# wizyoung/YOLOv3_TensorFlow

Hardware: NVIDIA H100
Metric: images/sec (higher is better)
Workload: dtype f16

## Files before the change

### include/yolob200.h

```cpp
#ifndef YOLOB200_H_
#define YOLOB200_H_

#include <stddef.h>
#include <stdint.h>

#ifdef __cplusplus
extern "C" {
#endif

typedef enum yb_status {
  YB_OK = 0,
  YB_ERR_INVALID_ARGUMENT = -1,
  YB_ERR_CUDA = -2,
  YB_ERR_UNSUPPORTED = -3,
  YB_ERR_WORKSPACE = -4
} yb_status;

typedef enum yb_dtype { YB_F16 = 0, YB_BF16 = 1, YB_F32 = 2, YB_E4M3 = 3 } yb_dtype;

typedef enum yb_wlayout {
  YB_W_HWIO = 0,
  YB_W_OIHW = 1,
  YB_W_OHWI = 2
} yb_wlayout;

int yb_version(void);
const char* yb_last_error_string(void);
int yb_set_option(const char* key, const char* value);
const char* yb_get_option(const char* key);
int yb_device_info(int* sm_count, int* cc_major, int* cc_minor);

typedef struct yb_conv_desc {
  int n, h, w;
  int cin, cout;
  int ksize;
  int stride;
  int in_ld;
  int out_ld;
  int res_ld;
  int dtype;
  int out_fp32;
  int leaky;
  int upsample2x;
} yb_conv_desc;

int yb_conv2d_fwd(const yb_conv_desc* d, const void* x, const void* w_packed, const float* scale,
                  const float* shift, const void* res, void* out, float* stat_sum, float* stat_sqsum,
                  void* stream);
int yb_conv_cout_pad(int cout);
int yb_conv2d_fwd_e4m3(const yb_conv_desc* d, const void* x, const void* w_packed, const float* scale,
                       const float* shift, const void* res, float res_scale, void* out, float out_scale, void* stream);
typedef struct yb_conv_schedule_info {
  int pingpong;
  int consumers;
  int cluster;
  int block_m, block_n, block_k;
  int stages;
  int num_kb;
  int num_m_tiles, num_n_tiles;
  int grid;
  int res_smem;
  int res_stages;
  int cluster_m;
  int cluster_n;
  int units;
  int epi_tma;
} yb_conv_schedule_info;
int yb_conv_schedule(const yb_conv_desc* d, int kh, int kw, int with_stats, int sm_count, yb_conv_schedule_info* info);

int yb_stem_conv_fwd(const float* x, const float* w_ohwi, const float* scale, const float* shift, int n, int h,
                     int w, int cout, int dtype, int leaky, void* out, void* stream);

int yb_conv3x3_thin_fwd(const yb_conv_desc* d, const void* x, const void* w_packed, const float* scale,
                        const float* shift, const void* res, void* out, void* stream);
int yb_stem_conv_fwd_tc(const float* x, const float* w_ohwi, const float* scale, const float* shift, int n, int h,
                        int w, int dtype, int leaky, void* out, void* stream);
int yb_stem_conv_fwd_tc_stats(const float* x, const float* w_ohwi, const float* scale, const float* shift, int n, int h,
                              int w, int dtype, int leaky, void* out, float* stat_sum, float* stat_sqsum, void* stream);

int yb_conv3x3_halo_supported(const yb_conv_desc* d);
int yb_conv3x3_halo_fwd(const yb_conv_desc* d, const void* x, const void* w_packed, const float* scale,
                        const float* shift, const void* res, void* out, void* stream);
int yb_stem_conv1_fused_fwd(const yb_conv_desc* d, const float* image, const float* stem_w_ohwi, const float* stem_scale,
                            const float* stem_shift, const void* w_packed, const float* scale, const float* shift, void* out,
                            void* stream);

int yb_process_box(const float* boxes, const int32_t* labels, const int32_t* counts, int n, int vmax, int img_w,
                   int img_h, int class_num, const float* anchors9x2, float* y_true_1, float* y_true_2,
                   float* y_true_3, void* stream);
int yb_letterbox_params(int src_h, int src_w, int new_h, int new_w, double* resize_ratio, int* resize_h, int* resize_w,
                        int* dh, int* dw);
int yb_letterbox_normalize(const uint8_t* bgr, int src_h, int src_w, long src_pitch_bytes, int new_h, int new_w,
                           float* out_rgb, void* stream);
int yb_resize_batch(const uint8_t* images, long images_bytes, const int64_t* desc_host, const int64_t* desc_dev, int n,
                    int new_h, int new_w, int letterbox, int interp, float* out_rgb, double* params, void* stream);
int yb_resize_boxes(float* boxes, const int32_t* counts, int n, int vmax, int box_ld, const int64_t* desc_dev, int new_h,
                    int new_w, int letterbox, void* stream);
int yb_restore_boxes(float* boxes, const int32_t* counts, int n, int slots, int box_ld, const double* params,
                     void* stream);

int yb_pack_conv_weights(const float* src, int layout, int cout, int cin, int ksize, int cout_pad, int dtype,
                         void* dst, void* stream);
int yb_pack_conv_weights_e4m3(const float* src, int layout, int cout, int cin, int ksize, int cout_pad, void* dst,
                              float* w_scale, void* stream);
int yb_amax(const void* x, long ld, long rows, int cols, int dtype, float* out, void* stream);
int yb_bn_fold(const float* gamma, const float* beta, const float* mean, const float* var, int c, float eps,
               float* scale, float* shift, void* stream);

int yb_conv2d_wgrad(const yb_conv_desc* d, const void* x, const void* dz, int dz_ld, int dz_dilated, float* dw,
                    void* stream);
int yb_stem_conv_wgrad(const float* x, const void* dz, int dtype, int n, int h, int w, float* dw, void* stream);
int yb_stem_conv_wgrad_tc(const float* x, const void* dz, int dtype, int n, int h, int w, float* dw, void* stream);
int yb_pack_dgrad_weights(const float* w_ohwi, int cout, int cin, int ksize, int k_cout, int cin_pad, int dtype,
                          void* dst, void* stream);
int yb_pack_dgrad_weights_s2(const float* w_ohwi, int cout, int cin, int k_cout, int cin_pad, int dtype, void* dst,
                             void* stream);
int yb_conv2d_dgrad_s2(const yb_conv_desc* fwd, const void* dz, int dz_ld, int k_cout, const void* w_dgrad_s2,
                       const void* res, int res_ld, void* dx, int dx_ld, void* stream);
typedef struct yb_wgrad_schedule_info {
  int bnw;
  int tp;
  int stages;
  int num_kb;
  int kb_per_split;
  int splits;
  int tiles;
  int grid_x, grid_y, grid_z;
} yb_wgrad_schedule_info;
int yb_wgrad_schedule(const yb_conv_desc* d, int sm_count, yb_wgrad_schedule_info* info);
int yb_bn_finalize(const float* sum, const float* sqsum, long count, int c, const float* gamma, const float* beta,
                   float eps, float decay, float* moving_mean, float* moving_var, float* scale, float* shift,
                   float* save_mean, float* save_invstd, void* stream);
int yb_bn_act_apply(const void* z, long z_ld, const float* scale, const float* shift, const void* res, long res_ld,
                    void* out, long out_ld, int n, int h, int w, int c, int dtype, int leaky, int upsample2x,
                    void* stream);
int yb_bn_stats_act_apply(const void* z, long z_ld, const float* sum, const float* sqsum, const float* gamma,
                          const float* beta, float eps, float decay, float* moving_mean, float* moving_var,
                          float* scale, float* shift, float* save_mean, float* save_invstd, const void* res,
                          long res_ld, void* out, long out_ld, int n, int h, int w, int c, int dtype, int leaky,
                          int upsample2x, void* stream);
typedef struct yb_bn_schedule_info {
  int cpt;
  int r;
  int blocks_per_sm;
  int cv;
  int lanes;
  long rows_per_block;
  int grid;
} yb_bn_schedule_info;
int yb_bn_schedule(long rows, int c, int sm_count, yb_bn_schedule_info* info);
int yb_bn_bwd_reduce_workspace_bytes(size_t* bytes);
// ... 178 lines not shown
```

### yolov3_tensorflow_b200/_lib.py

```python
from __future__ import annotations

import ctypes as C
import os

_HERE = os.path.dirname(os.path.abspath(__file__))
LIB_PATH = os.path.join(_HERE, "libyolob200.so")

YB_F16, YB_BF16, YB_F32, YB_E4M3 = 0, 1, 2, 3
YB_W_HWIO, YB_W_OIHW, YB_W_OHWI = 0, 1, 2
YB_OPT_SGD, YB_OPT_MOMENTUM, YB_OPT_RMSPROP, YB_OPT_ADAM = 0, 1, 2, 3
YB_TRAIN_FORWARD_ONLY, YB_TRAIN_BN_FROZEN, YB_TRAIN_NO_BACKWARD = 1, 2, 4
YB_PHASE_LOCAL, YB_PHASE_GLOBAL = 0, 1
YB_VOC_MAX_GT = 1024
YB_KMEANS_MAX_K = 32
YB_JPEG_BAD_MARKER, YB_JPEG_BAD_RST, YB_JPEG_BAD_CODE, YB_JPEG_BAD_INDEX, YB_JPEG_TRUNCATED = 1, 2, 4, 8, 16
YB_LAYER_IGEMM, YB_LAYER_HALO, YB_LAYER_FUSED_STEM, YB_LAYER_STEM, YB_LAYER_THIN = 1, 2, 3, 4, 5


class YoloB200Error(RuntimeError):
    pass


if not os.path.exists(LIB_PATH):
    raise ImportError(
        f"{LIB_PATH} not found: build it with ./build.sh (or python -c 'import __graft_entry__ as g; g.build()'). "
        "yolov3_tensorflow_b200 has no CPU/PyTorch fallback.")

lib = C.CDLL(LIB_PATH)

vp, i32, f32, sz = C.c_void_p, C.c_int, C.c_float, C.c_size_t


class ConvDesc(C.Structure):
    _fields_ = [(n, i32) for n in ("n", "h", "w", "cin", "cout", "ksize", "stride", "in_ld", "out_ld", "res_ld",
                                   "dtype", "out_fp32", "leaky", "upsample2x")]


class ConvSchedule(C.Structure):
    _fields_ = [(n, i32) for n in ("pingpong", "consumers", "cluster", "block_m", "block_n", "block_k", "stages", "num_kb",
                                   "num_m_tiles", "num_n_tiles", "grid", "res_smem", "res_stages", "cluster_m",
                                   "cluster_n", "units", "epi_tma")]


class LayerSchedule(C.Structure):
    _fields_ = [(n, i32) for n in ("igemm", "pingpong", "cluster_m", "cluster_n", "block_m", "block_n", "num_m_tiles",
                                   "num_n_tiles", "units", "max_clusters", "grid", "residual", "res_smem", "kernel",
                                   "epi_tma", "det_block_n")]


class WgradSchedule(C.Structure):
    _fields_ = [(n, i32) for n in ("bnw", "tp", "stages", "num_kb", "kb_per_split", "splits", "tiles", "grid_x",
                                   "grid_y", "grid_z")]


class BnSchedule(C.Structure):
    _fields_ = [(n, i32) for n in ("cpt", "r", "blocks_per_sm", "cv", "lanes")] + [("rows_per_block", C.c_long),
                                                                                    ("grid", i32)]


class LayerInfo(C.Structure):
    _fields_ = [(n, i32) for n in ("index", "cin", "cout", "ksize", "stride", "has_bn", "in_h", "in_w", "out_h",
                                   "out_w", "is_head", "scope_index", "upsample2x")]


class JpegInfo(C.Structure):
    _fields_ = [(n, i32) for n in ("height", "width", "src_height", "src_width", "components", "h_samp", "v_samp",
                                   "restart_interval", "orientation", "mode")]


class Optimizer(C.Structure):
    _fields_ = [("kind", i32)] + [(n, f32) for n in ("lr", "grad_scale", "momentum", "decay", "beta1", "beta2", "epsilon",
                                                      "weight_decay", "clip_norm")]


_SIGS = {
    "yb_version": ([], i32),
    "yb_last_error_string": ([], C.c_char_p),
    "yb_set_option": ([C.c_char_p, C.c_char_p], i32),
    "yb_get_option": ([C.c_char_p], C.c_char_p),
    "yb_device_info": ([C.POINTER(i32)] * 3, i32),
    "yb_conv2d_fwd": ([C.POINTER(ConvDesc), vp, vp, vp, vp, vp, vp, vp, vp, vp], i32),
    "yb_conv2d_fwd_e4m3": ([C.POINTER(ConvDesc), vp, vp, vp, vp, vp, f32, vp, f32, vp], i32),
    "yb_conv_cout_pad": ([i32], i32),
    "yb_conv_schedule": ([C.POINTER(ConvDesc), i32, i32, i32, i32, C.POINTER(ConvSchedule)], i32),
    "yb_stem_conv_fwd": ([vp, vp, vp, vp, i32, i32, i32, i32, i32, i32, vp, vp], i32),
    "yb_conv3x3_thin_fwd": ([C.POINTER(ConvDesc), vp, vp, vp, vp, vp, vp, vp], i32),
    "yb_conv3x3_halo_supported": ([C.POINTER(ConvDesc)], i32),
    "yb_conv3x3_halo_fwd": ([C.POINTER(ConvDesc), vp, vp, vp, vp, vp, vp, vp], i32),
    "yb_stem_conv1_fused_fwd": ([C.POINTER(ConvDesc), vp, vp, vp, vp, vp, vp, vp, vp, vp], i32),
    "yb_stem_conv_fwd_tc": ([vp, vp, vp, vp, i32, i32, i32, i32, i32, vp, vp], i32),
    "yb_stem_conv_fwd_tc_stats": ([vp, vp, vp, vp, i32, i32, i32, i32, i32, vp, vp, vp, vp], i32),
    "yb_process_box": ([vp, vp, vp, i32, i32, i32, i32, i32, C.POINTER(f32), vp, vp, vp, vp], i32),
    "yb_letterbox_params": ([i32, i32, i32, i32, C.POINTER(C.c_double), C.POINTER(i32), C.POINTER(i32), C.POINTER(i32), C.POINTER(i32)], i32),
    "yb_letterbox_normalize": ([vp, i32, i32, C.c_long, i32, i32, vp, vp], i32),
    "yb_resize_batch": ([vp, C.c_long, vp, vp, i32, i32, i32, i32, i32, vp, vp, vp], i32),
    "yb_resize_boxes": ([vp, vp, i32, i32, i32, vp, i32, i32, i32, vp], i32),
    "yb_restore_boxes": ([vp, vp, i32, i32, i32, vp, vp], i32),
    "yb_pack_conv_weights": ([vp, i32, i32, i32, i32, i32, i32, vp, vp], i32),
    "yb_pack_conv_weights_e4m3": ([vp, i32, i32, i32, i32, i32, vp, vp, vp], i32),
    "yb_amax": ([vp, C.c_long, C.c_long, i32, i32, vp, vp], i32),
    "yb_bn_fold": ([vp, vp, vp, vp, i32, f32, vp, vp, vp], i32),
    "yb_conv2d_wgrad": ([C.POINTER(ConvDesc), vp, vp, i32, i32, vp, vp], i32),
    "yb_stem_conv_wgrad": ([vp, vp, i32, i32, i32, i32, vp, vp], i32),
    "yb_stem_conv_wgrad_tc": ([vp, vp, i32, i32, i32, i32, vp, vp], i32),
    "yb_pack_dgrad_weights": ([vp, i32, i32, i32, i32, i32, i32, vp, vp], i32),
    "yb_pack_dgrad_weights_s2": ([vp, i32, i32, i32, i32, i32, vp, vp], i32),
    "yb_conv2d_dgrad_s2": ([vp, vp, i32, i32, vp, vp, i32, vp, i32, vp], i32),
    "yb_bn_finalize": ([vp, vp, C.c_long, i32, vp, vp, f32, f32, vp, vp, vp, vp, vp, vp, vp], i32),
    "yb_bn_act_apply": ([vp, C.c_long, vp, vp, vp, C.c_long, vp, C.c_long, i32, i32, i32, i32, i32, i32, i32, vp], i32),
    "yb_wgrad_schedule": ([C.POINTER(ConvDesc), i32, C.POINTER(WgradSchedule)], i32),
    "yb_bn_stats_act_apply": ([vp, C.c_long, vp, vp, vp, vp, f32, f32, vp, vp, vp, vp, vp, vp, vp, C.c_long, vp, C.c_long,
                               i32, i32, i32, i32, i32, i32, i32, vp], i32),
    "yb_bn_schedule": ([C.c_long, i32, i32, C.POINTER(BnSchedule)], i32),
    "yb_bn_bwd_reduce_workspace_bytes": ([C.POINTER(sz)], i32),
    "yb_bn_bwd_reduce": ([vp, C.c_long, vp, C.c_long, vp, vp, vp, vp, i32, i32, i32, i32, i32, i32, i32, vp, vp, vp, vp], i32),
    "yb_bn_bwd_apply": ([vp, C.c_long, vp, C.c_long, vp, vp, vp, vp, vp, vp, vp, i32, i32, i32, i32, i32, i32, i32, i32, vp, C.c_long, vp], i32),
    "yb_col_sum": ([vp, C.c_long, C.c_long, i32, i32, vp, vp], i32),
    "yb_col_stats": ([vp, C.c_long, C.c_long, i32, i32, vp, vp, vp], i32),
    "yb_reorg_layer": ([vp, i32, i32, i32, i32, i32, i32, C.POINTER(f32), vp, vp, vp, vp, vp], i32),
    "yb_predict": ([vp, vp, vp, i32, i32, i32, i32, C.POINTER(f32), vp, vp, vp, vp, vp], i32),
    "yb_nms_workspace_bytes": ([i32, i32, i32, i32, C.POINTER(sz)], i32),
    "yb_nms": ([vp, vp, i32, i32, i32, i32, f32, f32, vp, sz, vp, vp, vp, vp, vp, vp], i32),
    "yb_voc_match": ([vp, vp, vp, vp, i32, i32, vp, vp, vp, i32, i32, C.c_double, vp, C.c_long, C.c_long, vp, vp], i32),
    "yb_voc_ap_workspace_bytes": ([C.c_long, i32, C.POINTER(sz)], i32),
    "yb_voc_ap": ([vp, C.c_long, vp, i32, i32, vp, sz, vp, vp], i32),
    "yb_kmeans_workspace_bytes": ([C.c_long, i32, C.POINTER(sz)], i32),
    "yb_kmeans_assign": ([vp, C.c_long, vp, i32, vp, vp, vp, vp, sz, vp], i32),
    "yb_kmeans_median": ([vp, C.c_long, vp, vp, i32, vp, vp, sz, vp], i32),
    "yb_kmeans_avg_iou": ([vp, C.c_long, vp, i32, vp, vp, sz, vp], i32),
    "yb_jpeg_parse": ([vp, sz, C.POINTER(JpegInfo)], i32),
    "yb_jpeg_pack_bytes": ([C.POINTER(vp), C.POINTER(sz), i32, C.POINTER(sz)], i32),
    "yb_jpeg_pack": ([C.POINTER(vp), C.POINTER(sz), i32, vp, sz, vp], i32),
    "yb_jpeg_workspace_bytes": ([vp, i32, C.POINTER(sz), C.POINTER(sz)], i32),
    "yb_jpeg_decode": ([vp, vp, i32, vp, vp, vp, vp, sz, vp], i32),
    "yb_loss_workspace_bytes": ([i32, i32, i32, C.POINTER(sz)], i32),
    "yb_loss_layer": ([vp, vp, i32, i32, i32, i32, i32, i32, C.POINTER(f32), i32, i32, f32, f32, vp, sz, vp, vp, i32, i32, vp], i32),
    "yb_loss_finalize": ([vp, vp, vp], i32),
    "yb_box_iou": ([vp, vp, C.c_long, i32, vp, vp], i32),
    "yb_net_create": ([C.POINTER(vp), i32, i32, i32, i32, i32, i32], i32),
    "yb_net_destroy": ([vp], i32),
    "yb_net_num_layers": ([vp], i32),
    "yb_net_layer_info": ([vp, i32, C.POINTER(LayerInfo)], i32),
    "yb_net_layer_schedule": ([vp, i32, i32, C.POINTER(LayerSchedule)], i32),
    "yb_net_arena_bytes": ([vp, C.POINTER(sz), C.POINTER(sz)], i32),
    "yb_net_bind": ([vp, vp, sz, vp, sz, vp], i32),
    "yb_net_refold_bn": ([vp, vp], i32),
    "yb_net_set_conv_params": ([vp, i32, vp, i32, vp, vp, vp, vp, vp, vp], i32),
    "yb_net_forward": ([vp, vp, vp, vp, vp, vp], i32),
    "yb_net_detect_supported": ([vp], i32),
    "yb_net_detect_workspace_bytes": ([vp, i32, C.POINTER(sz)], i32),
    "yb_net_detect": ([vp, vp, C.POINTER(f32), i32, f32, f32, vp, sz, vp, vp, vp, vp, vp, vp, vp], i32),
    "yb_net_detect_phases": ([vp, vp, C.POINTER(f32), i32, f32, f32, vp, sz, vp, vp, vp, vp, vp, vp, i32, vp], i32),
    "yb_net_forward_layers": ([vp, vp, vp, vp, vp, i32, i32, vp], i32),
    "yb_net_train_fwd_bwd": ([vp, vp, vp, vp, vp, C.POINTER(f32), i32, i32, f32, f32, vp, vp, vp, vp, i32, vp], i32),
    "yb_net_train_backward": ([vp, vp, i32, i32, i32, vp], i32),
    "yb_net_grad_range": ([vp, i32, i32, C.POINTER(vp), C.POINTER(sz)], i32),
    "yb_net_train_forward_layer": ([vp, vp, i32, i32, i32, f32, vp, vp, vp, i32, vp], i32),
    "yb_net_train_loss": ([vp, vp, vp, vp, C.POINTER(f32), i32, i32, f32, vp, vp], i32),
    "yb_net_train_backward_layer": ([vp, vp, i32, i32, i32, i32, vp], i32),
    "yb_net_train_join": ([vp, vp], i32),
    "yb_net_bn_exchange_buffer": ([vp, i32, i32, C.POINTER(vp), C.POINTER(sz)], i32),
    "yb_net_grad_buffer": ([vp, C.POINTER(vp), C.POINTER(sz)], i32),
    "yb_net_train_update": ([vp, C.POINTER(Optimizer), vp], i32),
    "yb_net_train_reset_state": ([vp, i32, vp], i32),
    "yb_net_opt_state": ([vp, C.POINTER(vp), C.POINTER(sz), C.POINTER(i32), C.POINTER(vp)], i32),
    "yb_net_opt_norms": ([vp, C.POINTER(vp), C.POINTER(i32)], i32),
    "yb_net_set_trainable": ([vp, i32, i32, vp], i32),
# ... 47 lines not shown
```

### yolov3_tensorflow_b200/csrc/conv_igemm.cu

```cuda
#include <cudaTypedefs.h>
#include <math.h>
#include <stdlib.h>
#include <string.h>

#include <type_traits>

#include "common.cuh"
#include "conv.cuh"
#include "wgmma.cuh"

namespace yb {

static constexpr int WG_ROWS = 64;
static constexpr int RING_BYTES = 196 * 1024;
static constexpr int EPI_LD = 33;
static constexpr int EPI_FLOATS = WG_ROWS * EPI_LD;

template <int BN, int BKB, int NC, bool RES = false>
struct Cfg {
  static constexpr int BLOCK_M = WG_ROWS * NC;
  static constexpr int THREADS = 128 * (NC + 1);
  static constexpr int A_BYTES = BLOCK_M * BKB;
  static constexpr int B_BYTES = BN * BKB;
  static constexpr int STAGE_BYTES = A_BYTES + B_BYTES;
// ... 320 lines not shown
  const int cluster_id = blockIdx.x / cs, num_clusters = gridDim.x / cs;
  const int nunits = num_units<CM, CN>(p);
  const int kb_per_tap = p.cin / BK;
  const int num_kb = p.kh * p.kw * kb_per_tap;

  if (wg == 0) {
    if (threadIdx.x == 0) {
      const int a_rows = C::BLOCK_M / CN, b_rows = BN / cm;
      const int rm = (int)rank / CN, rn = (int)rank % CN;
      const uint16_t a_mask = (uint16_t)(((1u << CN) - 1u) << (rm * CN));
      uint16_t b_mask = 0;
      for (int i = 0; i < cm; ++i) b_mask |= (uint16_t)(1u << (i * CN + rn));
      int stage = 0;
      uint32_t phase = 0;
      for (int unit = cluster_id; unit < nunits; unit += num_clusters) {
        int m_idx, n_idx;
        unit_coords<CM, CN>(p, unit, rank, m_idx, n_idx);
        const int ma = m_idx * C::BLOCK_M + rn * a_rows;
        const int nb = n_idx * BN + rm * b_rows;
        const int q = ma % p.Q;
        const int pp = (ma / p.Q) % p.P;
        const int img = ma / (p.Q * p.P);
        const int w_base = q * p.stride - p.pad;
        const int h_base = pp * p.stride - p.pad;
        int c0 = 0, tw = 0, th = 0, kcol = 0;
        for (int kb = 0; kb < num_kb; ++kb) {
          mbar_wait(&empty_bar[stage], phase ^ 1);
          mbar_arrive_expect_tx(&full_bar[stage], C::STAGE_BYTES);
          uint8_t* a_dst = sA + stage * C::A_BYTES + rn * a_rows * BKB;
          uint8_t* b_dst = sB + stage * C::B_BYTES + rm * b_rows * BKB;
          if constexpr (CN > 1) {
            if (p.im2col)
              tma_load_im2col_4d_multicast(a_dst, &tmA, &full_bar[stage], c0, w_base, h_base, img, (uint16_t)tw,
                                           (uint16_t)th, a_mask);
            else
              tma_load_2d_multicast(a_dst, &tmA, &full_bar[stage], c0, ma, a_mask);
          } else {
            if (p.im2col)
              tma_load_im2col_4d(a_dst, &tmA, &full_bar[stage], c0, w_base, h_base, img, (uint16_t)tw, (uint16_t)th);
            else
              tma_load_2d(a_dst, &tmA, &full_bar[stage], c0, ma);
          }
          if (cm > 1) tma_load_2d_multicast(b_dst, &tmB, &full_bar[stage], kcol, nb, b_mask);
          else tma_load_2d(b_dst, &tmB, &full_bar[stage], kcol, nb);
          c0 += BK; kcol += BK;
          if (c0 == p.cin) { c0 = 0; if (++tw == p.kw) { tw = 0; ++th; } }
          if (++stage == C::STAGES) { stage = 0; phase ^= 1; }
        }
      }
    }
    if constexpr (RES) {
      if (threadIdx.x == 32) {
        uint32_t rphase[NC] = {};
        int j = 0;
        for (int unit = cluster_id; unit < nunits; unit += num_clusters, ++j) {
          int m_idx, n_idx;
          unit_coords<CM, CN>(p, unit, rank, m_idx, n_idx);
          const int m0 = m_idx * C::BLOCK_M, n0 = n_idx * BN;
          if (m0 >= p.M) continue;
          const int w = j & 1;
          mbar_wait(&res_empty[w], rphase[w] ^ 1);
          mbar_arrive_expect_tx(&res_full[w], C::RES_TILE_BYTES);
#pragma unroll
          for (int b = 0; b < BN / C::RES_BOX_COLS; ++b)
            tma_load_2d(sR + w * C::RES_TILE_BYTES + b * C::RES_BOX_BYTES, &p.tmR, &res_full[w], n0 + b * C::RES_BOX_COLS, m0);
          rphase[w] ^= 1;
        }
      }
    }
  } else {
    using Mma = typename ConvMma<T, BN>::type;
    constexpr bool kRegEpi = !PP && !TMA && !std::is_same<T, __nv_fp8_e4m3>::value;
    const int cw = wg - 1;
    const int t = threadIdx.x & 127;
    const int lane = t & 31;
    const int bar_id = 1 + cw;
    float* stg = s_epi + cw * EPI_FLOATS;
    float* sst = s_stat + cw * 2 * BN;
    float* sss = s_ss + cw * 2 * BN;
    if (p.stat_sum != nullptr)
      for (int c = t; c < 2 * BN; c += 128) sst[c] = 0.f;
    auto release = [&](int st) {
      __syncwarp();
      if (lane == 0) {
        if (cs == 1) {
          mbar_arrive(&empty_bar[st]);
        } else {
#pragma unroll
          for (int r = 0; r < 4; ++r)
            if (r < cs) mbar_arrive_remote(&empty_bar[st], (uint32_t)r);
        }
      }
    };
    float acc[NH][BN / 2];
    int stage = 0, prev = 0;
    uint32_t phase = 0;
    auto skip_unit = [&]() {
      const int s = stage + num_kb;
      phase ^= (uint32_t)((s / C::STAGES) & 1);
      stage = s % C::STAGES;
    };
    if (PP && cw == 1) skip_unit();
    int cur_n0 = -1, ss_n0 = -1;
    const uint32_t a_off = PP ? 0u : cw * WG_ROWS * BKB;
    const int unit_step = PP ? 2 * num_clusters : num_clusters;
    uint32_t res_phase = 0;
    const uint8_t* sres = sR + cw * C::RES_TILE_BYTES;
    for (int unit = cluster_id + (PP ? cw * num_clusters : 0); unit < nunits; unit += unit_step) {
      int m_idx, n_idx;
      unit_coords<CM, CN>(p, unit, rank, m_idx, n_idx);
      const int m0 = m_idx * C::BLOCK_M;
      const int n0 = n_idx * BN;
      if (PP && unit != cluster_id) named_bar_sync(MMA_TURN_BAR + cw, 256);
      for (int kb = 0; kb < num_kb; ++kb) {
        mbar_wait(&full_bar[stage], phase);
        const uint32_t a_addr = smem_u32(sA + stage * C::A_BYTES) + a_off;
        const uint32_t b_addr = smem_u32(sB + stage * C::B_BYTES);
#pragma unroll
        for (int h = 0; h < NH; ++h) wgmma_fence_operand(acc[h]);
        wgmma_fence();
#pragma unroll
        for (int k = 0; k < BKB / 32; ++k)
#pragma unroll
          for (int h = 0; h < NH; ++h)
            Mma::mma(acc[h], make_kmajor_desc(a_addr + h * WG_ROWS * BKB + k * 32, C::SBO, C::SWIZZLE),
                     make_kmajor_desc(b_addr + k * 32, C::SBO, C::SWIZZLE), (kb | k) != 0);
        wgmma_commit();
#pragma unroll
        for (int h = 0; h < NH; ++h) wgmma_fence_operand(acc[h]);
        wgmma_wait<1>();
        if (kb > 0) release(prev);
        prev = stage;
        if (++stage == C::STAGES) { stage = 0; phase ^= 1; }
      }
      if (PP && unit + num_clusters < nunits) named_bar_arrive(MMA_TURN_BAR + (cw ^ 1), 256);
      wgmma_wait<0>();
#pragma unroll
      for (int h = 0; h < NH; ++h) wgmma_fence_operand(acc[h]);
      release(prev);
      if (PP) skip_unit();

      if (p.stat_sum != nullptr && n0 != cur_n0) {
        if (cur_n0 >= 0) stat_flush<BN>(p, sst, cur_n0, t, bar_id);
        cur_n0 = n0;
      }
      if (n0 != ss_n0) {
        warpgroup_bar(bar_id);
        for (int c = t; c < BN; c += 128) {
          const bool in = !DET || c < p.cout;
          const float sc = p.scale && in ? __ldg(p.scale + n0 + c) : 1.f;
          const float sh = p.shift && in ? __ldg(p.shift + n0 + c) : 0.f;
          if constexpr (TMA) {
            sss[(c >> 1) * 4 + (c & 1)] = sc;
            sss[(c >> 1) * 4 + 2 + (c & 1)] = sh;
          } else {
            sss[c] = sc;
            sss[BN + c] = sh;
          }
        }
        warpgroup_bar(bar_id);
        ss_n0 = n0;
      }
      if constexpr (DET) {
        epilogue_detect<BN>(p, acc[0], m0 + cw * WG_ROWS, t, stg, sss, bar_id);
      } else if constexpr (TMA) {
        if (m0 < p.M) {
          const int wrow = 16 * (t >> 5);
// ... 125 lines not shown
  cuuint64_t strides[2] = {(cuuint64_t)w * 3 * 4, (cuuint64_t)h * w * 3 * 4};
  cuuint32_t box[3] = {(cuuint32_t)box_f, (cuuint32_t)box_h, 1};
  cuuint32_t estr[3] = {1, 1, 1};
  CUresult r = g_encode_tiled(tm, CU_TENSOR_MAP_DATA_TYPE_FLOAT32, 3, const_cast<float*>(base), dims, strides, box, estr,
                              CU_TENSOR_MAP_INTERLEAVE_NONE, CU_TENSOR_MAP_SWIZZLE_NONE, CU_TENSOR_MAP_L2_PROMOTION_L2_128B,
                              CU_TENSOR_MAP_FLOAT_OOB_FILL_NONE);
  if (r != CUDA_SUCCESS) {
    set_error("cuTensorMapEncodeTiled(image) failed (%d): n=%d h=%d w=%d box=%dx%d", (int)r, n, h, w, box_f, box_h);
    return YB_ERR_CUDA;
  }
  return YB_OK;
}

int make_tmap_tiled4d(CUtensorMap* tm, const void* base, int dtype, int n, int h, int w, int c, long ld, int box_c,
                      int box_w, int box_h, int estride) {
  int rc = load_driver_entry_points();
  if (rc) return rc;
  cuuint64_t dims[4] = {(cuuint64_t)c, (cuuint64_t)w, (cuuint64_t)h, (cuuint64_t)n};
  cuuint64_t strides[3] = {(cuuint64_t)ld * 2, (cuuint64_t)w * ld * 2, (cuuint64_t)h * w * ld * 2};
  cuuint32_t box[4] = {(cuuint32_t)box_c, (cuuint32_t)box_w, (cuuint32_t)box_h, 1};
  cuuint32_t estr[4] = {1, (cuuint32_t)estride, (cuuint32_t)estride, 1};
  CUtensorMapSwizzle sw = box_c * 2 == 128 ? CU_TENSOR_MAP_SWIZZLE_128B : CU_TENSOR_MAP_SWIZZLE_64B;
  CUresult r = g_encode_tiled(tm, tm_dtype(dtype), 4, const_cast<void*>(base), dims, strides, box, estr,
                              CU_TENSOR_MAP_INTERLEAVE_NONE, sw, CU_TENSOR_MAP_L2_PROMOTION_L2_128B,
                              CU_TENSOR_MAP_FLOAT_OOB_FILL_NONE);
  if (r != CUDA_SUCCESS) {
    set_error("cuTensorMapEncodeTiled(4d) failed (%d): n=%d h=%d w=%d c=%d ld=%ld box=%dx%dx%d stride %d", (int)r, n, h, w, c,
              ld, box_c, box_w, box_h, estride);
    return YB_ERR_CUDA;
  }
  return YB_OK;
}

int make_tmap_im2col_px(CUtensorMap* tm, const void* base, int dtype, int n, int h, int w, int c, long ld, int ksize,
                        int stride, int pad, int bk, int pixels);
int make_tmap_im2col(CUtensorMap* tm, const void* base, int dtype, int n, int h, int w, int c, long ld, int ksize,
                     int stride, int pad, int bk) {
  return make_tmap_im2col_px(tm, base, dtype, n, h, w, c, ld, ksize, stride, pad, bk, 128);
}
int make_tmap_im2col_px(CUtensorMap* tm, const void* base, int dtype, int n, int h, int w, int c, long ld, int ksize,
                        int stride, int pad, int bk, int pixels) {
  int rc = load_driver_entry_points();
  if (rc) return rc;
  cuuint64_t dims[4] = {(cuuint64_t)c, (cuuint64_t)w, (cuuint64_t)h, (cuuint64_t)n};
  const int es = tm_esize(dtype);
  cuuint64_t strides[3] = {(cuuint64_t)ld * es, (cuuint64_t)w * ld * es, (cuuint64_t)h * w * ld * es};
  int lower[2] = {-pad, -pad};
  int upper[2] = {pad - (ksize - 1), pad - (ksize - 1)};
  cuuint32_t estr[4] = {1, (cuuint32_t)stride, (cuuint32_t)stride, 1};
  CUtensorMapSwizzle sw = bk * es == 128 ? CU_TENSOR_MAP_SWIZZLE_128B : CU_TENSOR_MAP_SWIZZLE_64B;
  CUresult r = g_encode_im2col(tm, tm_dtype(dtype), 4, const_cast<void*>(base), dims, strides, lower, upper,
                               (cuuint32_t)bk, (cuuint32_t)pixels, estr, CU_TENSOR_MAP_INTERLEAVE_NONE, sw,
                               CU_TENSOR_MAP_L2_PROMOTION_L2_128B, CU_TENSOR_MAP_FLOAT_OOB_FILL_NONE);
  if (r != CUDA_SUCCESS) {
    set_error("cuTensorMapEncodeIm2col failed (%d): n=%d h=%d w=%d c=%d ld=%ld k=%d s=%d", (int)r, n, h, w, c, ld,
              ksize, stride);
    return YB_ERR_CUDA;
  }
  int drv = 0;
  cudaDriverGetVersion(&drv);
  if (drv <= 13010 && (size_t)n * h * w * ld * es < 131072) {
    reinterpret_cast<uint64_t*>(tm)[1] &= ~(1ull << 21);
  }
  return YB_OK;
}

int conv_units(const ConvParams& p) {
  return ceil_div(p.num_m_tiles, p.cluster / p.cluster_n) * (p.num_n_tiles / p.cluster_n);
}

int conv_grid(const ConvParams& p, int sms, int max_active) {
  const int cs = p.cluster;
  const int units = conv_units(p);
  int max_clusters = sms / cs;
  if (max_active > 0 && max_active < max_clusters) max_clusters = max_active;
  if (p.ctas > 0) {
    const int cap = p.ctas / cs > 1 ? p.ctas / cs : 1;
    if (cap < max_clusters) max_clusters = cap;
  }
  const int clusters = units < max_clusters ? units : max_clusters;
  return clusters * cs;
}

struct ClusterCapacity { int v[64][5] = {}; };
static int cluster_capacity(ClusterCapacity& cap, const void* kern, int threads, int smem, int cs, int* out) {
  int dev = 0;
  YB_CUDA(cudaGetDevice(&dev));
  int& v = cap.v[dev & 63][cs];
  if (v == 0) {
    cudaLaunchConfig_t cfg;
    memset(&cfg, 0, sizeof(cfg));
    cfg.gridDim = dim3(cs);
    cfg.blockDim = dim3(threads);
    cfg.dynamicSmemBytes = smem;
    cudaLaunchAttribute attr[1];
    attr[0].id = cudaLaunchAttributeClusterDimension;
    attr[0].val.clusterDim.x = cs; attr[0].val.clusterDim.y = 1; attr[0].val.clusterDim.z = 1;
    cfg.attrs = attr;
    cfg.numAttrs = 1;
    int n = 0;
    YB_CUDA(cudaOccupancyMaxActiveClusters(&n, kern, &cfg));
    if (n <= 0) { set_error("conv: no cluster of %d CTAs (%d bytes of shared memory each) fits the device", cs, smem); return YB_ERR_CUDA; }
    v = n;
  }
  *out = v;
  return YB_OK;
}

template <typename T, int BN, int BKB, int NC, bool DET = false, bool PP = false, int CM = 0, int CN = 1, bool RES = false,
          bool TMA = false>
struct ConvKernel {
  using C = Cfg<BN, BKB, NC, RES>;
  static constexpr auto kernel = conv_igemm_kernel<T, BN, BKB, NC, DET, PP, CM, CN, RES, TMA>;
};

static int no_conv_kernel(const ConvParams& p) {
  set_error("conv: no kernel for dtype %d, %d-column tiles, %d-byte k-blocks, %d consumer warpgroups, ping-pong %d, "
            "%d x %d cluster, shortcut tile %d, TMA-store epilogue %d, fused decode of %d columns", p.dtype, p.block_n,
            p.block_kb, p.consumers, p.pingpong, p.cluster / p.cluster_n, p.cluster_n, p.res_smem, p.epi_tma, p.det_e);
  return YB_ERR_UNSUPPORTED;
}

template <typename T, int BN, int BKB, bool RES, bool TMA, typename F>
static int conv_kernel_pp_shape(const ConvParams& p, F& f) {
  const int cn = p.cluster_n, cm = p.cluster / p.cluster_n;
  if (cm == 1 && cn == 1) return f(ConvKernel<T, BN, BKB, 2, false, true, 1, 1, RES, TMA>());
  if constexpr (sizeof(T) == 2) {
    if (cm == 2 && cn == 1) return f(ConvKernel<T, BN, BKB, 2, false, true, 2, 1, RES, TMA>());
    if (cm == 1 && cn == 2) return f(ConvKernel<T, BN, BKB, 2, false, true, 1, 2, RES, TMA>());
    if (cm == 2 && cn == 2) return f(ConvKernel<T, BN, BKB, 2, false, true, 2, 2, RES, TMA>());
  }
  return no_conv_kernel(p);
}
template <typename T, int BN, int BKB, bool RES, typename F>
static int conv_kernel_pp(const ConvParams& p, F& f) {
  if (!p.epi_tma) return conv_kernel_pp_shape<T, BN, BKB, RES, false>(p, f);
  if constexpr (sizeof(T) == 2) return conv_kernel_pp_shape<T, BN, BKB, RES, true>(p, f);
  return no_conv_kernel(p);
}

template <typename T, int BN, int BKB, bool DET, typename F>
static int conv_kernel_tile(const ConvParams& p, F& f) {
  constexpr bool b16 = sizeof(T) == 2;
  if (p.pingpong) {
    if constexpr (!DET) {
      if (!p.res_smem) return conv_kernel_pp<T, BN, BKB, false>(p, f);
      if constexpr (b16 && BN == 128 && BKB == 128) return conv_kernel_pp<T, BN, BKB, true>(p, f);
    }
    return no_conv_kernel(p);
  }
  const bool shape = p.cluster_n == 1 && (p.cluster == 1 || (b16 && (p.cluster == 2 || p.cluster == 4)));
  if (!shape || p.res_smem) return no_conv_kernel(p);
  if (p.consumers == 2 && !p.epi_tma) return f(ConvKernel<T, BN, BKB, 2, DET>());
  if constexpr (b16 && !DET) {
    if (p.consumers == 2) return f(ConvKernel<T, BN, BKB, 2, false, false, 0, 1, false, true>());
    if (p.consumers == 1 && !p.epi_tma) return f(ConvKernel<T, BN, BKB, 1>());
  }
  return no_conv_kernel(p);
}

template <typename T, typename F>
static int conv_kernel_type(const ConvParams& p, F& f) {
  const int bn = p.block_n, kb = p.block_kb;
  if (p.det_e) {
    if (bn == 64 && kb == 128) return conv_kernel_tile<T, 64, 128, true>(p, f);
    if (bn == 128 && kb == 128) return conv_kernel_tile<T, 128, 128, true>(p, f);
    if (bn == 256 && kb == 128) return conv_kernel_tile<T, 256, 128, true>(p, f);
    return no_conv_kernel(p);
  }
  if (bn == 128 && kb == 128) return conv_kernel_tile<T, 128, 128, false>(p, f);
  if (bn == 128 && kb == 64) return conv_kernel_tile<T, 128, 64, false>(p, f);
  if (bn == 64 && kb == 128) return conv_kernel_tile<T, 64, 128, false>(p, f);
  if (bn == 64 && kb == 64) return conv_kernel_tile<T, 64, 64, false>(p, f);
  return no_conv_kernel(p);
}

template <typename F>
static int conv_kernel_for(const ConvParams& p, F&& f) {
  if (p.dtype == YB_F16) return conv_kernel_type<__half>(p, f);
  if (p.dtype == YB_BF16) return conv_kernel_type<__nv_bfloat16>(p, f);
  if (p.dtype == YB_E4M3) return conv_kernel_type<__nv_fp8_e4m3>(p, f);
  return no_conv_kernel(p);
}

template <typename K>
static int conv_kernel_grid(const ConvParams& p, int* grid, int* max_clusters) {
  static DeviceOnce once;
  static ClusterCapacity capacity;
  const void* kern = reinterpret_cast<const void*>(K::kernel);
  int rc = ensure_smem_attr(once, kern, K::C::SMEM_BYTES);
  if (rc) return rc;
  *max_clusters = num_sms();
  if (p.cluster > 1) {
    rc = cluster_capacity(capacity, kern, K::C::THREADS, K::C::SMEM_BYTES, p.cluster, max_clusters);
    if (rc) return rc;
  }
  *grid = conv_grid(p, num_sms(), *max_clusters);
  return YB_OK;
}

int conv_launch(const ConvLaunch& l, cudaStream_t st) {
  const ConvParams& p = l.p;
  return conv_kernel_for(p, [&](auto k) -> int {
    using K = decltype(k);
    int grid = 0, max_clusters = 0;
    const int rc = conv_kernel_grid<K>(p, &grid, &max_clusters);
    if (rc) return rc;
    cudaLaunchConfig_t cfg;
    memset(&cfg, 0, sizeof(cfg));
    cfg.gridDim = dim3(grid);
    cfg.blockDim = dim3(K::C::THREADS);
    cfg.dynamicSmemBytes = K::C::SMEM_BYTES;
    cfg.stream = st;
    cudaLaunchAttribute attr[1];
    attr[0].id = cudaLaunchAttributeClusterDimension;
    attr[0].val.clusterDim.x = p.cluster; attr[0].val.clusterDim.y = 1; attr[0].val.clusterDim.z = 1;
    cfg.attrs = attr;
    cfg.numAttrs = 1;
    YB_CUDA(cudaLaunchKernelEx(&cfg, K::kernel, l.tmA, l.tmB, p));
    return YB_OK;
  });
}

int conv_launch_grid(const ConvParams& p, int* grid, int* max_clusters) {
  return conv_kernel_for(p, [&](auto k) -> int { return conv_kernel_grid<decltype(k)>(p, grid, max_clusters); });
}

static int conv_block_kb(int cin, int dtype) { return cin * tm_esize(dtype) % 128 == 0 ? 128 : 64; }

int conv_select(const ConvRequest& r, ConvParams* p) {
  memset(p, 0, sizeof(*p));
  const yb_conv_desc* d = &r.d;
  const bool win = r.kh != 0 || r.kw != 0;
  const int det = r.det_e;
  if (det && d->cout != 3 * det) {
    set_error("fused decode: %d output channels are not 3 x (5 + %d classes)", d->cout, det - 5);
    return YB_ERR_UNSUPPORTED;
  }
  YB_REQUIRE(det >= 0 && 3 * det <= 256, "fused decode: the %d columns of %d classes do not fit one 256-column tile "
             "(at most 80 classes; more take forward + predict + nms)", 3 * det, det - 5);
  if (win) {
    YB_REQUIRE(r.kh >= 1 && r.kh <= 2 && r.kw >= 1 && r.kw <= 2 && r.scatter >= 0 && r.scatter <= 4, "conv: bad window");
    YB_REQUIRE(d->stride == 1 && !d->out_fp32 && !d->upsample2x && !r.stats,
               "conv: windows are stride-1, 16-bit, non-upsampled and without statistics");
  }
  YB_REQUIRE(win || d->ksize == 1 || d->ksize == 3, "conv: ksize must be 1 or 3 (got %d)", d->ksize);
  YB_REQUIRE(d->stride == 1 || d->stride == 2, "conv: stride must be 1 or 2 (got %d)", d->stride);
  YB_REQUIRE(!(d->ksize == 1 && d->stride != 1), "conv: 1x1 stride-2 is not on the YOLOv3 path");
  YB_REQUIRE(d->cin % 32 == 0 && d->cin >= 32, "conv: cin must be a multiple of 32 (got %d); use yb_stem_conv_fwd", d->cin);
  YB_REQUIRE(d->dtype == YB_F16 || d->dtype == YB_BF16 || d->dtype == YB_E4M3, "conv: dtype must be f16, bf16 or e4m3");
  const bool e4m3 = d->dtype == YB_E4M3;
  if (e4m3) {
    YB_REQUIRE(d->cin % 64 == 0, "conv: e4m3 needs cin %% 64 == 0 (got %d)", d->cin);
    YB_REQUIRE(d->in_ld % 16 == 0 && (d->out_fp32 || d->out_ld % 16 == 0) && d->res_ld % 16 == 0,
               "conv: e4m3 needs in_ld, out_ld and res_ld to be multiples of 16");
    YB_REQUIRE(!win && !r.stats, "conv: e4m3 is a forward inference path (no windows, no statistics)");
    YB_REQUIRE(opt("YB_CONV_EG")[0] != '1' && opt("YB_CONV_MODE")[0] != '2' && opt("YB_CONV_EPI")[0] != 'r',
               "conv: e4m3 runs with two consumer warpgroups, no cluster and the staged epilogue "
               "(YB_CONV_EG, YB_CONV_MODE, YB_CONV_EPI are 16-bit only)");
  }
  YB_REQUIRE(d->h % d->stride == 0 && d->w % d->stride == 0, "conv: h,w must be divisible by stride");
  YB_REQUIRE(d->in_ld >= d->cin && d->in_ld % 8 == 0, "conv: in_ld %d invalid for cin %d", d->in_ld, d->cin);
  const int cout_pad = yb_conv_cout_pad(d->cout);
  if (!d->out_fp32) {
    YB_REQUIRE(d->cout % 32 == 0, "conv: 16-bit output needs cout %% 32 == 0 (got %d)", d->cout);
    YB_REQUIRE(d->out_ld >= d->cout && d->out_ld % 8 == 0, "conv: out_ld %d invalid", d->out_ld);
  } else {
    YB_REQUIRE(d->out_ld >= d->cout, "conv: out_ld %d invalid", d->out_ld);
  }
  const int P = d->h / d->stride, Q = d->w / d->stride;
  const int kh = win ? r.kh : d->ksize, kw = win ? r.kw : d->ksize;
  const int pad = win ? 0 : d->ksize / 2;
  const int bn = det ? (3 * det <= 64 ? 64 : 3 * det <= 128 ? 128 : 256) : (cout_pad % 128 == 0 ? 128 : 64);
  p->M = d->n * P * Q; p->P = P; p->Q = Q;
  p->consumers = (!det && opt("YB_CONV_EG")[0] == '1') ? 1 : 2;
  p->cluster = (!det && opt("YB_CONV_MODE")[0] == '2') ? (opt("YB_CONV_MC")[0] == '1' ? 4 : 2) : 1;
  const char* eo = opt("YB_CONV_EPI");
  YB_REQUIRE(eo[0] == '\0' || strcmp(eo, "reg") == 0 || strcmp(eo, "stage") == 0 || strcmp(eo, "tma") == 0,
             "conv: YB_CONV_EPI must be reg, stage or tma (got '%s')", eo);
  p->epi_reg = (!det && !r.stats && eo[0] == 'r') ? 1 : 0;
  p->ctas = opt_int("YB_CONV_CTAS", 0);
  const char* pp = opt("YB_CONV_PP");
  const bool pp_shape = pp[0] == '1' || (pp[0] != '0' && (kh * kw > 1 || bn != 128));
  p->pingpong = (!det && p->consumers == 2 && p->cluster == 1 && !p->epi_reg && pp_shape) ? 1 : 0;
  const int block_m = 64 * p->consumers;
  p->num_m_tiles = ceil_div(p->M, block_m);
  p->num_n_tiles = det ? 1 : cout_pad / bn;
  p->cluster_n = 1;
  if (p->pingpong && !e4m3) {
    const char* mc = opt("YB_CONV_MCAST");
    int cm = 1, cn = 1;
    if (mc[0] != '\0' && mc[0] != '0') {
      YB_REQUIRE((mc[0] == '1' || mc[0] == '2') && mc[1] == 'x' && (mc[2] == '1' || mc[2] == '2') && mc[3] == '\0',
                 "conv: YB_CONV_MCAST must be 0, 2x1, 1x2 or 2x2 (got '%s')", mc);
      cm = mc[0] - '0'; cn = mc[2] - '0';
    } else if (mc[0] == '\0' && r.plan_rule && kh * kw > 1) {
      cm = 2; cn = 2;
    }
    if (p->num_n_tiles % 2 != 0) cn = 1;
    p->cluster = cm * cn;
    p->cluster_n = cn;
  }
  const char* ro = opt("YB_CONV_RES");
  YB_REQUIRE(ro[0] == '\0' || strcmp(ro, "ldg") == 0 || strcmp(ro, "smem") == 0,
             "conv: YB_CONV_RES must be ldg or smem (got '%s')", ro);
  p->dtype = d->dtype;
  p->block_n = bn;
  p->block_kb = conv_block_kb(d->cin, d->dtype);
  p->det_e = det;
  p->res_smem = (r.res && p->pingpong && !e4m3 && !det && bn == 128 && p->block_kb == 128 && !r.scatter &&
                 !d->upsample2x && !d->out_fp32 && strcmp(ro, "ldg") != 0) ? 1 : 0;
  p->epi_tma = ((eo[0] == 't' || (eo[0] == '\0' && r.plan_rule)) && !e4m3 && !det && !r.stats && p->consumers == 2 &&
                !d->out_fp32 && !d->upsample2x && !win && (!r.res || p->res_smem)) ? 1 : 0;
  p->cout = d->cout; p->cin = d->cin; p->ksize = d->ksize; p->stride = d->stride; p->pad = pad;
  p->kh = kh; p->kw = kw; p->scatter = r.scatter;
  p->im2col = kh * kw > 1;
  p->out_fp32 = d->out_fp32; p->leaky = d->leaky; p->upsample = d->upsample2x;
  p->res_scale = 1.f; p->out_inv_scale = 1.f;
  return conv_kernel_for(*p, [](auto) -> int { return YB_OK; });
}

int conv_prepare(const ConvRequest& r, const void* x, const void* w_packed, const float* scale, const float* shift,
                 const void* res, void* out, float* stat_sum, float* stat_sqsum, ConvLaunch* l) {
  ConvParams* p = &l->p;
  int rc = conv_select(r, p);
  if (rc) return rc;
  const yb_conv_desc* d = &r.d;
  YB_REQUIRE(x && w_packed && out && (scale == nullptr) == (shift == nullptr), "conv: null pointer");
  YB_REQUIRE(((uintptr_t)x & 15) == 0 && ((uintptr_t)w_packed & 15) == 0 && ((uintptr_t)out & 15) == 0 &&
                 ((uintptr_t)res & 15) == 0,
             "conv: pointers must be 16-byte aligned");
  YB_REQUIRE((res != nullptr) == r.res, "conv: a residual pointer is given exactly when the request has a residual");
  if (res) YB_REQUIRE(d->res_ld >= d->cout && d->res_ld % 8 == 0 && !d->out_fp32, "conv: res_ld %d invalid", d->res_ld);
  YB_REQUIRE((stat_sum == nullptr) == (stat_sqsum == nullptr), "conv: stat_sum/stat_sqsum must both be given");
  YB_REQUIRE((stat_sum != nullptr) == r.stats, "conv: statistics pointers are given exactly when the request has them");
  const int cout_pad = yb_conv_cout_pad(d->cout);
  const int bk = p->block_kb / tm_esize(d->dtype);
  const int kh = p->kh, kw = p->kw;
  const int a_rows = 64 * p->consumers / p->cluster_n;
  const int b_rows = p->block_n / (p->cluster / p->cluster_n);
  p->scale = scale; p->shift = shift;
  p->out = out; p->out_ld = d->out_ld; p->res = res; p->res_ld = d->res_ld;
  p->stat_sum = stat_sum; p->stat_sqsum = stat_sqsum;
  if (p->res_smem) {
    rc = make_tmap_2d(&p->tmR, res, d->dtype, p->M, d->cout, d->res_ld, 64 * p->consumers, 64, 0);
    if (rc) return rc;
  }
  if (p->epi_tma) {
    rc = make_tmap_2d(&p->tmO, out, d->dtype, p->M, d->cout, d->out_ld, 16, 64, 0);
    if (rc) return rc;
  }
  if (p->im2col) {
    const bool win = r.kh != 0 || r.kw != 0;
    rc = make_tmap_im2col_px(&l->tmA, x, d->dtype, d->n, d->h, d->w, d->cin, d->in_ld, win ? 1 : d->ksize, d->stride,
                             p->pad, bk, a_rows);
  } else {
    rc = make_tmap_2d(&l->tmA, x, d->dtype, (long)d->n * d->h * d->w, d->cin, d->in_ld, a_rows, bk, 0);
  }
  if (rc) return rc;
  return make_tmap_2d(&l->tmB, w_packed, d->dtype, cout_pad, (long)kh * kw * d->cin, (long)kh * kw * d->cin, b_rows, bk,
                      1);
}

int conv_prepare_dgrad_s2(const yb_conv_desc* fwd, const void* dz, int dz_ld, int k_cout, const void* w_dgrad_s2,
                          const void* res, int res_ld, void* dx, int dx_ld, ConvLaunch* l) {
  YB_REQUIRE(fwd && dz && w_dgrad_s2 && dx, "dgrad_s2: null pointer");
  YB_REQUIRE(fwd->ksize == 3 && fwd->stride == 2 && fwd->h % 2 == 0 && fwd->w % 2 == 0, "dgrad_s2: 3x3 stride-2 convs only");
  YB_REQUIRE(k_cout >= fwd->cout && k_cout % 32 == 0 && dz_ld >= k_cout, "dgrad_s2: dz must hold k_cout (multiple of 32) channels");
  ConvRequest r{*fwd};
  yb_conv_desc& d = r.d;
  d.h = fwd->h / 2; d.w = fwd->w / 2; d.cin = k_cout; d.cout = fwd->cin; d.ksize = 1; d.stride = 1;
  d.in_ld = dz_ld; d.out_ld = dx_ld; d.res_ld = res_ld; d.out_fp32 = 0; d.leaky = 0; d.upsample2x = 0;
  r.res = res != nullptr;
  const int cin_pad = yb_conv_cout_pad(fwd->cin);
  for (int c = 0; c < 4; ++c) {
    r.kh = 1 + (c >> 1); r.kw = 1 + (c & 1); r.scatter = 1 + c;
    const uint8_t* w = static_cast<const uint8_t*>(w_dgrad_s2) + dgrad_s2_class_offset(c, cin_pad, k_cout) * 2;
    int rc = conv_prepare(r, dz, w, nullptr, nullptr, res, dx, nullptr, nullptr, &l[c]);
    if (rc) return rc;
  }
  return YB_OK;
}

}

extern "C" int yb_conv_cout_pad(int cout) { return (cout + 63) / 64 * 64; }

extern "C" int yb_conv_schedule(const yb_conv_desc* d, int kh, int kw, int with_stats, int sm_count,
                                yb_conv_schedule_info* info) {
  YB_REQUIRE(d && info && sm_count > 0, "conv_schedule: bad argument");
  yb::ConvRequest r{*d};
  r.kh = kh; r.kw = kw; r.stats = with_stats != 0;
  yb::ConvParams p, pr;
  int rc = yb::conv_select(r, &p);
  if (rc) return rc;
  r.res = true;
  rc = yb::conv_select(r, &pr);
  if (rc) return rc;
  auto stages = [](const yb::ConvParams& q, int* s) {
    return yb::conv_kernel_for(q, [&](auto k) -> int { *s = decltype(k)::C::STAGES; return YB_OK; });
  };
  rc = stages(p, &info->stages);
  if (rc) return rc;
  rc = stages(pr, &info->res_stages);
  if (rc) return rc;
  info->res_smem = pr.res_smem;
  info->epi_tma = p.epi_tma;
  info->pingpong = p.pingpong;
  info->consumers = p.consumers;
  info->cluster = p.cluster;
  info->block_m = 64 * p.consumers;
  info->block_n = p.block_n;
  info->block_k = p.block_kb / yb::tm_esize(d->dtype);
  info->num_kb = p.kh * p.kw * d->cin / info->block_k;
  info->num_m_tiles = p.num_m_tiles;
  info->num_n_tiles = p.num_n_tiles;
  info->grid = yb::conv_grid(p, sm_count, 0);
  info->cluster_m = p.cluster / p.cluster_n;
  info->cluster_n = p.cluster_n;
  info->units = yb::conv_units(p);
  return YB_OK;
}

extern "C" int yb_conv2d_fwd(const yb_conv_desc* d, const void* x, const void* w_packed, const float* scale,
                             const float* shift, const void* res, void* out, float* stat_sum, float* stat_sqsum,
                             void* stream) {
  if (!d) { yb::set_error("conv: null descriptor"); return YB_ERR_INVALID_ARGUMENT; }
  yb::ConvRequest r{*d};
  r.stats = stat_sum != nullptr;
  r.res = res != nullptr;
  yb::ConvLaunch l;
  int rc = yb::conv_prepare(r, x, w_packed, scale, shift, res, out, stat_sum, stat_sqsum, &l);
  if (rc) return rc;
  return yb::conv_launch(l, static_cast<cudaStream_t>(stream));
}

extern "C" int yb_conv2d_fwd_e4m3(const yb_conv_desc* d, const void* x, const void* w_packed, const float* scale,
                                  const float* shift, const void* res, float res_scale, void* out, float out_scale,
                                  void* stream) {
  YB_REQUIRE(d && d->dtype == YB_E4M3, "conv_e4m3: descriptor dtype must be YB_E4M3");
  YB_REQUIRE(res_scale > 0.f && out_scale > 0.f && isfinite(res_scale) && isfinite(out_scale),
             "conv_e4m3: scales must be positive and finite");
  yb::ConvRequest r{*d};
  r.res = res != nullptr;
  yb::ConvLaunch l;
  int rc = yb::conv_prepare(r, x, w_packed, scale, shift, res, out, nullptr, nullptr, &l);
  if (rc) return rc;
  l.p.res_scale = res_scale;
  l.p.out_inv_scale = 1.f / out_scale;
  return yb::conv_launch(l, static_cast<cudaStream_t>(stream));
}

extern "C" int yb_conv2d_dgrad_s2(const yb_conv_desc* fwd, const void* dz, int dz_ld, int k_cout, const void* w_dgrad_s2,
                                  const void* res, int res_ld, void* dx, int dx_ld, void* stream) {
  yb::ConvLaunch l[4];
  int rc = yb::conv_prepare_dgrad_s2(fwd, dz, dz_ld, k_cout, w_dgrad_s2, res, res_ld, dx, dx_ld, l);
  for (int c = 0; c < 4 && rc == YB_OK; ++c) rc = yb::conv_launch(l[c], static_cast<cudaStream_t>(stream));
  return rc;
}
```

Before: 6981.

## Add 8-CTA multicast clusters and route plan-rule 1x1 TMA convs to pingpong

Adds 4x1, 4x2 and 2x4 cluster instantiations of the pingpong conv kernel. For 8-CTA clusters the empty-barrier release now spreads remote arrivals across eight lanes. The n-cluster size is halved until it divides the tile count. Plan-rule 1x1 convs with a TMA-eligible epilogue are now routed to the pingpong path, which by default also brings them multicast eligibility. A query entry point for the maximum number of active clusters is exposed. The default multicast stays 2x2, so the 8-CTA shapes only run when selected through an option.

```diff
diff --git a/include/yolob200.h b/include/yolob200.h
--- a/include/yolob200.h
+++ b/include/yolob200.h
@@ -67,6 +67,8 @@
   int epi_tma;
 } yb_conv_schedule_info;
 int yb_conv_schedule(const yb_conv_desc* d, int kh, int kw, int with_stats, int sm_count, yb_conv_schedule_info* info);
+int yb_conv_max_active_clusters(int dtype, int cluster_m, int cluster_n, int res_smem, int epi_tma, int* max_clusters,
+                                int* smem_bytes);
 
 int yb_stem_conv_fwd(const float* x, const float* w_ohwi, const float* scale, const float* shift, int n, int h,
                      int w, int cout, int dtype, int leaky, void* out, void* stream);
diff --git a/yolov3_tensorflow_b200/_lib.py b/yolov3_tensorflow_b200/_lib.py
--- a/yolov3_tensorflow_b200/_lib.py
+++ b/yolov3_tensorflow_b200/_lib.py
@@ -83,6 +83,7 @@
     "yb_conv2d_fwd_e4m3": ([C.POINTER(ConvDesc), vp, vp, vp, vp, vp, f32, vp, f32, vp], i32),
     "yb_conv_cout_pad": ([i32], i32),
     "yb_conv_schedule": ([C.POINTER(ConvDesc), i32, i32, i32, i32, C.POINTER(ConvSchedule)], i32),
+    "yb_conv_max_active_clusters": ([i32, i32, i32, i32, i32, C.POINTER(i32), C.POINTER(i32)], i32),
     "yb_stem_conv_fwd": ([vp, vp, vp, vp, i32, i32, i32, i32, i32, i32, vp, vp], i32),
     "yb_conv3x3_thin_fwd": ([C.POINTER(ConvDesc), vp, vp, vp, vp, vp, vp, vp], i32),
     "yb_conv3x3_halo_supported": ([C.POINTER(ConvDesc)], i32),
diff --git a/yolov3_tensorflow_b200/csrc/conv_igemm.cu b/yolov3_tensorflow_b200/csrc/conv_igemm.cu
--- a/yolov3_tensorflow_b200/csrc/conv_igemm.cu
+++ b/yolov3_tensorflow_b200/csrc/conv_igemm.cu
@@ -426,7 +426,9 @@
       for (int c = t; c < 2 * BN; c += 128) sst[c] = 0.f;
     auto release = [&](int st) {
       __syncwarp();
-      if (lane == 0) {
+      if constexpr (CM * CN == 8) {
+        if (lane < 8) mbar_arrive_remote(&empty_bar[st], (uint32_t)lane);
+      } else if (lane == 0) {
         if (cs == 1) {
           mbar_arrive(&empty_bar[st]);
         } else {
@@ -718,7 +720,7 @@
   return clusters * cs;
 }
 
-struct ClusterCapacity { int v[64][5] = {}; };
+struct ClusterCapacity { int v[64][9] = {}; };
 static int cluster_capacity(ClusterCapacity& cap, const void* kern, int threads, int smem, int cs, int* out) {
   int dev = 0;
   YB_CUDA(cudaGetDevice(&dev));
@@ -765,6 +767,9 @@
     if (cm == 2 && cn == 1) return f(ConvKernel<T, BN, BKB, 2, false, true, 2, 1, RES, TMA>());
     if (cm == 1 && cn == 2) return f(ConvKernel<T, BN, BKB, 2, false, true, 1, 2, RES, TMA>());
     if (cm == 2 && cn == 2) return f(ConvKernel<T, BN, BKB, 2, false, true, 2, 2, RES, TMA>());
+    if (cm == 4 && cn == 1) return f(ConvKernel<T, BN, BKB, 2, false, true, 4, 1, RES, TMA>());
+    if (cm == 4 && cn == 2) return f(ConvKernel<T, BN, BKB, 2, false, true, 4, 2, RES, TMA>());
+    if (cm == 2 && cn == 4) return f(ConvKernel<T, BN, BKB, 2, false, true, 2, 4, RES, TMA>());
   }
   return no_conv_kernel(p);
 }
@@ -917,7 +922,9 @@
   p->epi_reg = (!det && !r.stats && eo[0] == 'r') ? 1 : 0;
   p->ctas = opt_int("YB_CONV_CTAS", 0);
   const char* pp = opt("YB_CONV_PP");
-  const bool pp_shape = pp[0] == '1' || (pp[0] != '0' && (kh * kw > 1 || bn != 128));
+  const bool plan_tma_1x1 = r.plan_rule && eo[0] == '\0' && !e4m3 && !det && !r.stats && !r.res && !d->out_fp32 &&
+                            !d->upsample2x && !win;
+  const bool pp_shape = pp[0] == '1' || (pp[0] != '0' && (kh * kw > 1 || bn != 128 || plan_tma_1x1));
   p->pingpong = (!det && p->consumers == 2 && p->cluster == 1 && !p->epi_reg && pp_shape) ? 1 : 0;
   const int block_m = 64 * p->consumers;
   p->num_m_tiles = ceil_div(p->M, block_m);
@@ -927,13 +934,15 @@
     const char* mc = opt("YB_CONV_MCAST");
     int cm = 1, cn = 1;
     if (mc[0] != '\0' && mc[0] != '0') {
-      YB_REQUIRE((mc[0] == '1' || mc[0] == '2') && mc[1] == 'x' && (mc[2] == '1' || mc[2] == '2') && mc[3] == '\0',
-                 "conv: YB_CONV_MCAST must be 0, 2x1, 1x2 or 2x2 (got '%s')", mc);
+      const bool ok = mc[1] == 'x' && mc[3] == '\0' &&
+                      (((mc[0] == '1' || mc[0] == '2') && (mc[2] == '1' || mc[2] == '2')) ||
+                       (mc[0] == '4' && mc[2] == '2') || (mc[0] == '2' && mc[2] == '4'));
+      YB_REQUIRE(ok, "conv: YB_CONV_MCAST must be 0, 2x1, 1x2 or 2x2, or 4x2 or 2x4 for 8-CTA clusters (got '%s')", mc);
       cm = mc[0] - '0'; cn = mc[2] - '0';
     } else if (mc[0] == '\0' && r.plan_rule && kh * kw > 1) {
       cm = 2; cn = 2;
     }
-    if (p->num_n_tiles % 2 != 0) cn = 1;
+    while (p->num_n_tiles % cn != 0) cn /= 2;
     p->cluster = cm * cn;
     p->cluster_n = cn;
   }
@@ -1058,6 +1067,23 @@
   return YB_OK;
 }
 
+extern "C" int yb_conv_max_active_clusters(int dtype, int cluster_m, int cluster_n, int res_smem, int epi_tma,
+                                           int* max_clusters, int* smem_bytes) {
+  YB_REQUIRE((dtype == YB_F16 || dtype == YB_BF16) && cluster_m >= 1 && cluster_n >= 1 && max_clusters && smem_bytes,
+             "conv_max_active_clusters: bad argument");
+  yb::ConvParams p;
+  memset(&p, 0, sizeof(p));
+  p.dtype = dtype; p.block_n = 128; p.block_kb = 128; p.consumers = 2; p.pingpong = 1;
+  p.cluster = cluster_m * cluster_n; p.cluster_n = cluster_n; p.res_smem = res_smem != 0; p.epi_tma = epi_tma != 0;
+  p.num_m_tiles = cluster_m; p.num_n_tiles = cluster_n;
+  return yb::conv_kernel_for(p, [&](auto k) -> int {
+    using K = decltype(k);
+    int grid = 0;
+    *smem_bytes = K::C::SMEM_BYTES;
+    return yb::conv_kernel_grid<K>(p, &grid, max_clusters);
+  });
+}
+
 extern "C" int yb_conv2d_fwd(const yb_conv_desc* d, const void* x, const void* w_packed, const float* scale,
                              const float* shift, const void* res, void* out, float* stat_sum, float* stat_sqsum,
                              void* stream) {
```

Result: no change. 7009, median of 6 (+0.4%).
